# vivek-tiwari-vt/2048-Using-Reinforcement-Learning

Hardware: AMD Instinct MI355X
Metric: board-steps/sec (batched env.step) (higher is better)
Workload: dtype u8 (packed log2 tiles; f64 reward arithmetic, f32 reward out)

## Files before the change

2048-using-reinforcement-learning_amd/csrc/g2048_board.h:

```cpp
#pragma once
#include <stdint.h>

#if defined(__HIPCC__)
#include <hip/hip_runtime.h>
#define G2048_HD __device__ __forceinline__
#define G2048_PERM(s0, s1, sel) __builtin_amdgcn_perm((s0), (s1), (sel))
#define G2048_UDOT4(a, b, c) __builtin_amdgcn_udot4((a), (b), (c), false)
#else
#define G2048_HD inline
#if !defined(G2048_PERM) || !defined(G2048_UDOT4)
#error "host builds of g2048_board.h (test harness only) must define G2048_PERM and G2048_UDOT4"
#endif
#endif

namespace g2048 {

struct Board { uint32_t w[4]; };

constexpr uint32_t B80 = 0x80808080u;
constexpr uint32_t B7F = 0x7f7f7f7fu;

enum : uint32_t { DOM_STEP = 1, DOM_RESET = 2, DOM_BEAM = 3, DOM_SYNTH_BOARD = 4, DOM_SYNTH_ACTION = 5, DOM_EPISODE = 6, DOM_POLICY = 7,
                  DOM_SIMULATE = 8, DOM_MINIBATCH = 9, DOM_REPLAY = 10 };

// ... 199 lines not shown
        uint32_t g;
        const Board d = move_agent(b, 3u, g, false);
        m = (m & 7u) | (same(d, b) ? 0u : 8u);
    }
    return m;
}

G2048_HD bool game_over(const Board &b) { return valid_mask_env(b) == 0u; }

G2048_HD uint32_t spawn_rowprefix(Board &b, uint32_t h, bool enable = true, uint32_t *zf_out = nullptr)
{
    const uint32_t ones = 0x01010101u;
    const uint32_t z0 = zflag(b.w[0]), z1 = zflag(b.w[1]), z2 = zflag(b.w[2]), z3 = zflag(b.w[3]);
    const uint32_t c0 = popc(z0), c1 = c0 + popc(z1), c2 = c1 + popc(z2), n = c2 + popc(z3);
    const uint32_t idx = ((h >> 16) * n) >> 16;
    const uint32_t row = (idx >= c0 ? 1u : 0u) + (idx >= c1 ? 1u : 0u) + (idx >= c2 ? 1u : 0u);
    const uint32_t z = row == 0 ? z0 : row == 1 ? z1 : row == 2 ? z2 : z3;
    const uint32_t k1 = idx + 1u - (row == 0 ? 0u : row == 1 ? c0 : row == 2 ? c1 : c2);
    const uint32_t hit = zflag(((z >> 7) * ones) ^ (enable ? k1 * ones : 0x7f7f7f7fu)) & z;
    const uint32_t add = hit >> (((h & 0xffffu) >= 58982u) ? 6 : 7);
    b.w[0] |= row == 0 ? add : 0u; b.w[1] |= row == 1 ? add : 0u;
    b.w[2] |= row == 2 ? add : 0u; b.w[3] |= row == 3 ? add : 0u;
    if (zf_out) {
        zf_out[0] = z0 ^ (row == 0 ? hit : 0u); zf_out[1] = z1 ^ (row == 1 ? hit : 0u);
        zf_out[2] = z2 ^ (row == 2 ? hit : 0u); zf_out[3] = z3 ^ (row == 3 ? hit : 0u);
    }
    return n;
}

G2048_HD uint32_t spawn_prefix(Board &b, uint32_t h, bool enable = true, uint32_t *zf_out = nullptr)
{
    const uint32_t ones = 0x01010101u;
    const uint32_t z0 = zflag(b.w[0]), z1 = zflag(b.w[1]), z2 = zflag(b.w[2]), z3 = zflag(b.w[3]);
    const uint32_t p0 = (z0 >> 7) * ones, p1 = (z1 >> 7) * ones, p2 = (z2 >> 7) * ones, p3 = (z3 >> 7) * ones;
    const uint32_t c0 = p0 >> 24, c1 = c0 + (p1 >> 24), c2 = c1 + (p2 >> 24), n = c2 + (p3 >> 24);
    const uint32_t idx = ((h >> 16) * n) >> 16;
    uint32_t t_on = (idx + 1u) * ones;
#if defined(__HIPCC__)
    asm volatile("" : "+v"(t_on));
#endif
    const uint32_t target = enable ? t_on : 0x7f7f7f7fu;
    const uint32_t h0 = zflag(p0 ^ target) & z0;
    const uint32_t h1 = zflag((p1 + c0 * ones) ^ target) & z1;
    const uint32_t h2 = zflag((p2 + c1 * ones) ^ target) & z2;
    const uint32_t h3 = zflag((p3 + c2 * ones) ^ target) & z3;
    const uint32_t sh = ((h & 0xffffu) >= 58982u) ? 6u : 7u;
    b.w[0] |= h0 >> sh; b.w[1] |= h1 >> sh; b.w[2] |= h2 >> sh; b.w[3] |= h3 >> sh;
    if (zf_out) { zf_out[0] = z0 ^ h0; zf_out[1] = z1 ^ h1; zf_out[2] = z2 ^ h2; zf_out[3] = z3 ^ h3; }
    return n;
}

G2048_HD Board fresh_board(uint32_t h0, uint32_t h1)
{
    const uint32_t cell0 = h0 >> 28;
    uint32_t cell1 = ((h1 >> 16) * 15u) >> 16;
    cell1 += cell1 >= cell0 ? 1u : 0u;
    const uint32_t code0 = (h0 & 0xffffu) >= 58982u ? 2u : 1u, code1 = (h1 & 0xffffu) >= 58982u ? 2u : 1u;
    const uint32_t t0 = code0 << (8u * (cell0 & 3u)), t1 = code1 << (8u * (cell1 & 3u));
    const uint32_t r0 = cell0 >> 2, r1 = cell1 >> 2;
    Board b;
#pragma unroll
    for (uint32_t r = 0; r < 4; ++r) b.w[r] = (r0 == r ? t0 : 0u) | (r1 == r ? t1 : 0u);
    return b;
}

G2048_HD uint32_t rng_draw(uint32_t k0, uint32_t k1, uint64_t id, uint32_t ctr)
{
    uint32_t h = (uint32_t)id ^ k0;
    h ^= h >> 16; h *= 0x85EBCA6Bu; h ^= h >> 13; h *= 0xC2B2AE35u; h ^= h >> 16;
    h += k1 + (uint32_t)(id >> 32) * 0x9E3779B1u + ctr * 0x85EBCA77u;
    h ^= h >> 16; h *= 0x7FEB352Du; h ^= h >> 15; h *= 0x846CA68Bu; h ^= h >> 16;
    return h;
}

G2048_HD uint32_t rng_draw_lo(uint32_t k0, uint32_t k1h, uint32_t id_lo, uint32_t ctr)
{
    uint32_t h = id_lo ^ k0;
    h ^= h >> 16; h *= 0x85EBCA6Bu; h ^= h >> 13; h *= 0xC2B2AE35u; h ^= h >> 16;
// ... 67 lines not shown
    const uint32_t v01 = geflag(cur.w[1], cur.w[0]) & n0 & n1;
    const uint32_t v12 = geflag(cur.w[2], cur.w[1]) & n1 & n2;
    const uint32_t v23 = geflag(cur.w[3], cur.w[2]) & n2 & n3;
    const uint32_t colcnt = (v01 >> 7) + (v12 >> 7) + (v23 >> 7);
#pragma unroll
    for (int i = 0; i < 4; ++i) {
        const uint32_t x = cur.w[i], n = i == 0 ? n0 : i == 1 ? n1 : i == 2 ? n2 : n3;
        const uint32_t h = geflag(x >> 8, x) & n & (n >> 8);
        const uint32_t c = popc(h) + ((colcnt >> (8 * i)) & 0xffu);
        r += (double)c * 0.1;
    }
    return r;
}

G2048_HD double reward_env(const Board &cur, const TileStats &st, uint32_t gain, bool valid,
                           uint32_t empty_before, uint32_t empty_after)
{
    return reward_env_from((double)gain / 4.0, cur, st, valid, empty_before, empty_after);
}

struct TenthByProduct {
    static constexpr uint32_t kColShift = 7u;
    G2048_HD double operator()(uint32_t rows, uint32_t cols) const { return (double)(rows + cols) * 0.1; }
    G2048_HD double crowded(double r, uint32_t empty_after) const { return empty_after <= 2u ? r - 2.0 : r; }
};

#define G2048_TENTHS 8
#define G2048_TENTHS_INIT { 0.0 * 0.1, 1.0 * 0.1, 2.0 * 0.1, 3.0 * 0.1, 4.0 * 0.1, 5.0 * 0.1, 6.0 * 0.1, 7.0 * 0.1 }
#define G2048_CROWDED 17
#define G2048_CROWDED_INIT { -2.0, -2.0, -2.0, 0.0, 0.0, 0.0, 0.0, 0.0, 0.0, 0.0, 0.0, 0.0, 0.0, 0.0, 0.0, 0.0, 0.0 }

template <class TENTH = TenthByProduct>
G2048_HD double reward_env_folded(const Board &cur, const TileStats &st, uint32_t gain, bool valid,
                                  uint32_t empty_before, uint32_t empty_after, TENTH tenth = TENTH())
{
    const int32_t q = (int32_t)gain - (valid ? 0 : 8) + 2 * ((int32_t)empty_after - (int32_t)empty_before);
    double r = (double)q * 0.25;
    r += div_small_ints((double)st.edge, (double)st.total) * 1.0;
    r = tenth.crowded(r, empty_after);
    const uint32_t n0 = nzflag(cur.w[0]), n1 = nzflag(cur.w[1]), n2 = nzflag(cur.w[2]), n3 = nzflag(cur.w[3]);
    const uint32_t v01 = geflag(cur.w[1], cur.w[0]) & n0 & n1;
    const uint32_t v12 = geflag(cur.w[2], cur.w[1]) & n1 & n2;
    const uint32_t v23 = geflag(cur.w[3], cur.w[2]) & n2 & n3;
    const uint32_t colcnt = (v01 >> TENTH::kColShift) + (v12 >> TENTH::kColShift) + (v23 >> TENTH::kColShift);
#pragma unroll
    for (int i = 0; i < 4; ++i) {
        const uint32_t x = cur.w[i], n = i == 0 ? n0 : i == 1 ? n1 : i == 2 ? n2 : n3;
        const uint32_t h = geflag(x >> 8, x) & n & (n >> 8);
        r += tenth(popc(h), (colcnt >> (8 * i)) & 0xffu);
    }
    return r;
}

G2048_HD uint32_t pair_count(const Board &b);
G2048_HD bool game_over_counted(const Board &b, uint32_t n_empty)
{
#if defined(__HIPCC__)
    const bool full = n_empty == 0u;
    uint32_t pairs = 1u;
    if (__builtin_amdgcn_ballot_w64(full) != 0ull) pairs = pair_count(b);
    return n_empty == 16u || (full && pairs == 0u);
#else
    if (n_empty == 16u) return true;
    if (n_empty != 0u) return false;
    return pair_count(b) == 0u;
#endif
}

struct StepOut { Board board; uint32_t gain; double reward; uint32_t flags; };

template <class MOVE, class TENTH = TenthByProduct>
G2048_HD StepOut step_board_with(const Board &prev, MOVE move, uint32_t h, TENTH tenth = TENTH())
{
    StepOut o;
    uint32_t merges;
    Board cur = move(prev, o.gain, merges);
    const bool valid = !same(cur, prev);
    uint32_t empty_mid;
    uint32_t zf[4];
    empty_mid = spawn_prefix(cur, h, valid, zf);
    const uint32_t empty_before = empty_mid - merges;
    const uint32_t empty_after = empty_mid - (valid ? 1u : 0u);
    const TileStats st = tile_stats_z(cur, empty_after, zf[0], zf[1], zf[2], zf[3]);
    o.reward = reward_env_folded(cur, st, o.gain, valid, empty_before, empty_after, tenth);
    const bool done = game_over_counted(cur, empty_after);
    const uint32_t maxcode = 31u - (uint32_t)__builtin_clz(st.orbits | 1u);
    o.flags = (done ? 1u : 0u) | (valid ? 2u : 0u) | (maxcode << 3);
    o.board = cur;
    return o;
}

G2048_HD StepOut step_board(const Board &prev, uint32_t action, uint32_t h)
{
    return step_board_with(prev, [action](const Board &b, uint32_t &g, uint32_t &m) { return move_env(b, action, g, m); }, h);
}

template <class TENTH = TenthByProduct>
G2048_HD StepOut step_board_sel_noop(const Board &prev, const DirSel &sel, bool noop, uint32_t h, TENTH tenth = TENTH())
{
    return step_board_with(prev, [&sel, noop](const Board &b, uint32_t &g, uint32_t &m) {
        const Board r = move_env_sel(b, sel, g, m);
        g = noop ? 0u : g; m = noop ? 0u : m;
        return Board{{noop ? b.w[0] : r.w[0], noop ? b.w[1] : r.w[1], noop ? b.w[2] : r.w[2], noop ? b.w[3] : r.w[3]}};
    }, h, tenth);
}

template <class TENTH = TenthByProduct>
G2048_HD StepOut step_board_sel(const Board &prev, const DirSel &sel, uint32_t h, TENTH tenth = TENTH())
{
    return step_board_with(prev, [&sel](const Board &b, uint32_t &g, uint32_t &m) { return move_env_sel(b, sel, g, m); }, h, tenth);
}

G2048_HD uint32_t sample_action(float p0, float p1, float p2, float p3, uint32_t mask4, uint32_t h, float &prob)
{
    const uint32_t m = (mask4 & 15u) ? (mask4 & 15u) : 15u;
    const float w0 = (m & 1u) ? p0 + 1e-10f : 0.0f, w1 = (m & 2u) ? p1 + 1e-10f : 0.0f;
    const float w2 = (m & 4u) ? p2 + 1e-10f : 0.0f, w3 = (m & 8u) ? p3 + 1e-10f : 0.0f;
// ... 275 lines not shown
```

2048-using-reinforcement-learning_amd/csrc/g2048_kernels.hip:

```cpp
#include <hip/hip_runtime.h>
#include <hip/hip_fp16.h>
#include <stddef.h>

#include "../../include/g2048.h"
#include "../../include/g2048_testing.h"
#include "g2048_board.h"
#include "g2048_host.h"
#include "g2048_instrument.h"
#include "g2048_rng.h"

using namespace g2048;

namespace {

enum { KB_STEP = 0, KB_EPISODE = 2, KB_BEAM = 4, KB_POLICY = 6, KB_INDEX = 8 };

constexpr int kBlock = 256;
constexpr int kStepBoardsPerLane = 1;

__device__ const uint32_t kDirTable[G2048_DIR_TABLE_WORDS] = G2048_DIR_TABLE_INIT;

#include "g2048_step_table.h"

__device__ __forceinline__ void dir_table_to_lds(uint4 *s_dir)
{
    const uint32_t l = threadIdx.x & (G2048_DIR_TABLE_WORDS - 1u);
    reinterpret_cast<uint32_t *>(s_dir)[l] = kDirTable[l];
}

__device__ __forceinline__ DirSel dir_sel(const uint4 *s_dir, uint32_t action)
{
    const uint4 i = s_dir[2u * action], o = s_dir[2u * action + 1u];
    return DirSel{i.x, i.y, i.z, i.w, o.x, o.y, o.z, o.w};
}

__device__ __forceinline__ Board load_board(const uint4 *p, size_t i)
{
    const uint4 v = p[i];
    return Board{{v.x, v.y, v.z, v.w}};
}

__device__ __forceinline__ void store_board(uint4 *p, size_t i, const Board &b)
// ... 484 lines not shown

__global__ void keys_advance_kernel(uint32_t *keyblock, unsigned long long *counter, uint64_t seed)
{
    const uint64_t idx = *counter;
    const Keys s = rng_keys(seed, DOM_STEP, idx), e = rng_keys(seed, DOM_EPISODE, idx);
    const Keys b = rng_keys(seed, DOM_BEAM, idx), p = rng_keys(seed, DOM_POLICY, idx);
    keyblock[KB_STEP] = s.k0; keyblock[KB_STEP + 1] = s.k1; keyblock[KB_EPISODE] = e.k0; keyblock[KB_EPISODE + 1] = e.k1;
    keyblock[KB_BEAM] = b.k0; keyblock[KB_BEAM + 1] = b.k1; keyblock[KB_POLICY] = p.k0; keyblock[KB_POLICY + 1] = p.k1;
    keyblock[KB_INDEX] = (uint32_t)idx; keyblock[KB_INDEX + 1] = (uint32_t)(idx >> 32);
    *counter = idx + 1ull;
}

__global__ void selftest_kernel(uint32_t *result, uint32_t a, uint32_t b, double x, double y, double z)
{
    uint32_t bad = 0;
    if (perm(a, b, 0x07040300u) != (((a >> 24) << 24) | ((a & 0xffu) << 16) | ((b >> 24) << 8) | (b & 0xffu))) bad |= 1u;
    if (perm(a, b, 0x0c0c0c05u) != ((a >> 8) & 0xffu)) bad |= 2u;
    if (dot4(a, b, 7u) != 7u + (a & 0xffu) * (b & 0xffu) + ((a >> 8) & 0xffu) * ((b >> 8) & 0xffu) +
                              ((a >> 16) & 0xffu) * ((b >> 16) & 0xffu) + (a >> 24) * (b >> 24)) bad |= 4u;
    if (x * y + z != 0.0) bad |= 8u;
    const Board c = {{0x03020100u, 0x07060504u, 0x0b0a0908u, 0x0f0e0d0cu}};
    const Board t = transpose(c);
    if (t.w[0] != 0x0c080400u || t.w[1] != 0x0d090501u || t.w[2] != 0x0e0a0602u || t.w[3] != 0x0f0b0703u) bad |= 16u;
    const Board r = rot180(c);
    if (r.w[0] != 0x0c0d0e0fu || r.w[3] != 0x00010203u) bad |= 32u;
    *result = bad;
}

struct StepBound {
    const uint4 *in; const uint8_t *actions; uint4 *out; uint32_t *score; void *reward; uint8_t *flags;
    size_t n; uint32_t id_lo, id_hi_term;
};

struct StepCall { uint64_t magic; StepBound b; uint64_t seed; uint32_t opts, per_lane, grid, reserved; };
static_assert(sizeof(StepCall) <= G2048_STEP_CALL_BYTES, "the caller's block holds a StepCall");
constexpr uint64_t kStepCallMagic = 0x6b63617038343032ull;

constexpr uint32_t kStepOpts = G2048_STEP_REWARD_F64 | G2048_STEP_AUTO_RESET | G2048_STEP_RANDOM_ACTIONS | G2048_STEP_NOOP_ACTIONS |
                               (3u << G2048_STEP_TUNE_SHIFT);

int step_check(const char *what, const void *boards_in, const uint8_t *actions, const void *boards_out, const uint32_t *score_inout,
               const void *reward_out, const uint8_t *flags_out, uint32_t opts)
{
    const bool random_actions = (opts & G2048_STEP_RANDOM_ACTIONS) != 0u;
    if (!boards_in || (!actions && !random_actions) || !boards_out || !score_inout || !reward_out || !flags_out)
        return fail(G2048_ERR_ARG, "%s: null pointer", what);
    if (!aligned(boards_in, 16) || !aligned(boards_out, 16)) return fail(G2048_ERR_ARG, "%s: board arrays must be 16-byte aligned", what);
    if (!aligned(score_inout, 4) || !aligned(reward_out, (opts & G2048_STEP_REWARD_F64) ? 8 : 4))
        return fail(G2048_ERR_ARG, "%s: score/reward arrays misaligned", what);
    if (opts & ~kStepOpts) return fail(G2048_ERR_ARG, "%s: unknown opts 0x%x", what, opts);
    if (((opts >> G2048_STEP_TUNE_SHIFT) & 3u) == 3u)
        return fail(G2048_ERR_ARG, "%s: tune 3 (four boards per lane) was removed: measured slower at every size", what);
    return G2048_OK;
}

int step_boards_per_lane(uint32_t opts, size_t n)
{
    const unsigned tune = (opts >> G2048_STEP_TUNE_SHIFT) & 3u;
    return tune == 1 ? 1 : tune == 2 ? 2 : (n >= ((size_t)1 << 22) ? 2 : kStepBoardsPerLane);
}

template <class Kernel>
void launch_step(Kernel kernel, unsigned grid, hipStream_t s, const StepBound &b, const uint32_t *keyblock, const Keys &k, const Keys &e,
                 uint32_t a0 = 0, uint32_t a1 = 0)
{
    hipLaunchKernelGGL(kernel, dim3(grid), dim3(kBlock), 0, s, b.n, keyblock, b.in, b.actions, b.score, b.id_lo, b.id_hi_term, k.k0, k.k1, b.out,
                       b.reward, b.flags, e.k0, e.k1, a0, a1);
}

void launch_plain_step(bool f64, bool ar, int per_lane, unsigned grid, hipStream_t s, const StepBound &b, const uint32_t *keyblock,
                       const Keys &k, const Keys &e);

}

extern "C" {

const char *g2048_last_error(void) { return g_err; }
int g2048_abi_version(void) { return G2048_ABI_VERSION; }
unsigned g2048_build_flags(void) { return kInstrument; }

int g2048_device_count(void)
{
    int n = 0;
    if (hipGetDeviceCount(&n) != hipSuccess) { (void)hipGetLastError(); return 0; }
    return n;
}

static int step_impl(const void *boards_in, const uint8_t *actions, void *boards_out, uint32_t *score_inout,
                     void *reward_out, uint8_t *flags_out, uint64_t seed, uint64_t step_index,
                     uint64_t board_id_base, size_t n, uint32_t opts, void *stream, const uint32_t *keyblock)
{
    if (n == 0) return G2048_OK;
    const bool random_actions = (opts & G2048_STEP_RANDOM_ACTIONS) != 0u;
    if (const int rc = step_check("g2048_step", boards_in, actions, boards_out, score_inout, reward_out, flags_out, opts)) return rc;
    {
        const uint64_t to_wrap = 0x100000000ull - (board_id_base & 0xffffffffull);
        if ((uint64_t)n > to_wrap) {
            const size_t n1 = (size_t)to_wrap, rb = (opts & G2048_STEP_REWARD_F64) ? 8u : 4u;
            const int rc = step_impl(boards_in, actions, boards_out, score_inout, reward_out, flags_out, seed, step_index, board_id_base, n1,
                                     opts, stream, keyblock);
            if (rc != G2048_OK) return rc;
            return step_impl(static_cast<const char *>(boards_in) + 16u * n1, actions ? actions + n1 : nullptr,
                             static_cast<char *>(boards_out) + 16u * n1, score_inout + n1, static_cast<char *>(reward_out) + rb * n1,
                             flags_out + n1, seed, step_index, board_id_base + n1, n - n1, opts, stream, keyblock);
// ... 1 lines not shown
    }
    if (random_actions && keyblock) return fail(G2048_ERR_ARG, "g2048_step_dyn: RANDOM_ACTIONS needs the scalar form");
    const Keys k = rng_keys(seed, DOM_STEP, step_index), e = rng_keys(seed, DOM_EPISODE, step_index);
    hipStream_t s = static_cast<hipStream_t>(stream);
    const StepBound b = {static_cast<const uint4 *>(boards_in), actions, static_cast<uint4 *>(boards_out), score_inout, reward_out, flags_out,
                         n, (uint32_t)board_id_base, rng_hi_term(board_id_base)};
    const bool f64 = opts & G2048_STEP_REWARD_F64, ar = opts & G2048_STEP_AUTO_RESET;
    const int per_lane = step_boards_per_lane(opts, n);
    if (opts & G2048_STEP_NOOP_ACTIONS) {
        if (random_actions) return fail(G2048_ERR_ARG, "g2048_step: NOOP_ACTIONS needs explicit actions");
        with_bools(f64, ar, [&](auto F, auto A) {
            launch_step(step_kernel<decltype(F)::value, decltype(A)::value, 1, kBlock, false, true>, blocks_for(n, kBlock), s, b, keyblock, k, e);
        });
    } else if (random_actions) {
        const Keys ak = rng_keys(seed, DOM_SYNTH_ACTION, step_index);
        with_bools(f64, ar, [&](auto F, auto A) {
            launch_step(step_kernel<decltype(F)::value, decltype(A)::value, 1, kBlock, true>, blocks_for(n, kBlock), s, b, keyblock, k, e, ak.k0, ak.k1);
        });
    } else {
        launch_plain_step(f64, ar, per_lane, blocks_for(n, (size_t)kBlock * per_lane), s, b, keyblock, k, e);
    }
    return check_launch("g2048_step");
}

namespace {
void launch_plain_step(bool f64, bool ar, int per_lane, unsigned grid, hipStream_t s, const StepBound &b, const uint32_t *keyblock,
                       const Keys &k, const Keys &e)
{
    with_bools(f64, ar, [&](auto F, auto A) {
        if (per_lane == 1) launch_step(step_kernel<decltype(F)::value, decltype(A)::value, 1, kBlock>, grid, s, b, keyblock, k, e);
        else launch_step(step_kernel<decltype(F)::value, decltype(A)::value, 2, kBlock>, grid, s, b, keyblock, k, e);
    });
}
}

int g2048_step(const void *boards_in, const uint8_t *actions, void *boards_out, uint32_t *score_inout,
               void *reward_out, uint8_t *flags_out, uint64_t seed, uint64_t step_index,
               uint64_t board_id_base, size_t n, uint32_t opts, void *stream)
{
    return step_impl(boards_in, actions, boards_out, score_inout, reward_out, flags_out, seed, step_index, board_id_base, n,
                     opts, stream, nullptr);
}

int g2048_step_pack(const void *boards_in, const uint8_t *actions, void *boards_out, uint32_t *score_inout, void *reward_out,
                    uint8_t *flags_out, uint64_t seed, uint64_t board_id_base, size_t n, uint32_t opts, void *call_out)
{
    if (!call_out || !aligned(call_out, 8)) return fail(G2048_ERR_ARG, "g2048_step_pack: call_out must be an 8-byte aligned block of G2048_STEP_CALL_BYTES");
    static_cast<StepCall *>(call_out)->magic = 0;
    if (const int rc = step_check("g2048_step_pack", boards_in, actions, boards_out, score_inout, reward_out, flags_out, opts)) return rc;
    if (opts & (G2048_STEP_RANDOM_ACTIONS | G2048_STEP_NOOP_ACTIONS))
        return fail(G2048_ERR_ARG, "g2048_step_pack: RANDOM_ACTIONS and NOOP_ACTIONS go through g2048_step");
    if ((uint64_t)n > 0x100000000ull - (board_id_base & 0xffffffffull))
        return fail(G2048_ERR_ARG, "g2048_step_pack: the board ids cross a multiple of 2^32 (two launches): use g2048_step");
    const int per_lane = step_boards_per_lane(opts, n);
    StepCall c = {};
    c.b = StepBound{static_cast<const uint4 *>(boards_in), actions, static_cast<uint4 *>(boards_out), score_inout, reward_out, flags_out,
                    n, (uint32_t)board_id_base, rng_hi_term(board_id_base)};
    c.seed = seed; c.opts = opts; c.per_lane = (uint32_t)per_lane; c.grid = blocks_for(n, (size_t)kBlock * per_lane);
    c.magic = kStepCallMagic;
    *static_cast<StepCall *>(call_out) = c;
    return G2048_OK;
}

int g2048_step_packed(const void *call, uint64_t step_index, void *stream)
{
    const StepCall *c = static_cast<const StepCall *>(call);
    if (!c || !aligned(c, 8) || c->magic != kStepCallMagic) return fail(G2048_ERR_ARG, "g2048_step_packed: not a block g2048_step_pack filled");
    if (c->b.n == 0) return G2048_OK;
    launch_plain_step(c->opts & G2048_STEP_REWARD_F64, c->opts & G2048_STEP_AUTO_RESET, (int)c->per_lane, c->grid, static_cast<hipStream_t>(stream),
                      c->b, nullptr, rng_keys(c->seed, DOM_STEP, step_index), rng_keys(c->seed, DOM_EPISODE, step_index));
    return check_launch("g2048_step_packed");
}

int g2048_step_dyn(const void *boards_in, const uint8_t *actions, void *boards_out, uint32_t *score_inout,
                   void *reward_out, uint8_t *flags_out, const uint32_t *keyblock, uint64_t board_id_base, size_t n,
                   uint32_t opts, void *stream)
{
    if (!keyblock) return fail(G2048_ERR_ARG, "g2048_step_dyn: null key block");
    return step_impl(boards_in, actions, boards_out, score_inout, reward_out, flags_out, 0, 0, board_id_base, n, opts, stream,
                     keyblock);
}

int g2048_step_many(const void *boards_in, const uint8_t *actions_stream_or_null, void *boards_out, uint32_t *score_inout,
                    void *reward_stream_out_or_null, uint8_t *flags_stream_out_or_null, uint8_t *flags_last_out,
                    uint32_t *episodes_out_or_null, uint64_t seed, uint64_t step_index0, uint32_t steps,
                    uint64_t board_id_base, size_t n, uint32_t opts, void *stream)
{
    if (n == 0) return G2048_OK;
    if (!boards_in || !boards_out || !score_inout || !flags_last_out) return fail(G2048_ERR_ARG, "g2048_step_many: null pointer");
    if (!aligned(boards_in, 16) || !aligned(boards_out, 16)) return fail(G2048_ERR_ARG, "g2048_step_many: board arrays must be 16-byte aligned");
    const bool f64 = (opts & G2048_STEP_REWARD_F64) != 0u, ar = (opts & G2048_STEP_AUTO_RESET) != 0u;
    const bool random_actions = (opts & G2048_STEP_RANDOM_ACTIONS) != 0u;
    if (!aligned(score_inout, 4) || !aligned(episodes_out_or_null, 4) || !aligned(reward_stream_out_or_null, f64 ? 8 : 4))
        return fail(G2048_ERR_ARG, "g2048_step_many: score / reward / episode arrays misaligned");
    if (!random_actions && !actions_stream_or_null)
        return fail(G2048_ERR_ARG, "g2048_step_many: no policy: pass an actions stream or set G2048_STEP_RANDOM_ACTIONS");
    if (opts & ~(G2048_STEP_REWARD_F64 | G2048_STEP_AUTO_RESET | G2048_STEP_RANDOM_ACTIONS)) return fail(G2048_ERR_ARG, "g2048_step_many: unknown opts 0x%x", opts);
    if (steps == 0) return fail(G2048_ERR_ARG, "g2048_step_many: steps must be at least 1");
    hipStream_t s = static_cast<hipStream_t>(stream);
    const auto launch = [&](auto kernel) {
        hipLaunchKernelGGL(kernel, dim3(blocks_for(n, kBlock)), dim3(kBlock), 0, s, static_cast<const uint4 *>(boards_in), actions_stream_or_null,
                           static_cast<uint4 *>(boards_out), score_inout, reward_stream_out_or_null, flags_stream_out_or_null, flags_last_out,
                           episodes_out_or_null, seed, step_index0, steps, board_id_base, n);
    };
// ... 281 lines not shown
```

2048-using-reinforcement-learning_amd/g2048/_build.py:

```python
import os
import shutil
import subprocess
import sys

CSRC = os.path.join(os.path.dirname(os.path.dirname(os.path.abspath(__file__))), "csrc")
INCLUDE = os.path.join(CSRC, "..", "..", "include")
LIBRARIES = {
    "": ("libg2048_hip.so", "G2048_LIB",
         ["g2048_kernels.hip", "g2048_beam.hip", "g2048_rollout.hip", "g2048_policy.hip", "g2048_tpolicy.hip", "g2048_qnet.hip",
          "g2048_qnet_batch.hip", "g2048_qnet_grad.hip", "g2048_qnet_step.hip", "g2048_per.hip", "g2048_ppo_grad.hip", "g2048_ppo_step.hip"],
         ["g2048.h", "g2048_testing.h"]),
    "TRAIN_": ("libg2048_train_hip.so", "G2048_TRAIN_LIB", ["g2048_qnet_train.hip"], ["g2048_train.h"]),
    "TLEARN_": ("libg2048_tlearn_hip.so", "G2048_TLEARN_LIB", ["g2048_tpolicy_grad.hip"], ["g2048_tlearn.h"]),
    "TSTEP_": ("libg2048_tstep_hip.so", "G2048_TSTEP_LIB", ["g2048_tpolicy_step.hip"], ["g2048_tstep.h"]),
    "TTRAIN_": ("libg2048_ttrain_hip.so", "G2048_TTRAIN_LIB", ["g2048_tpolicy_train.hip"], ["g2048_ttrain.h"]),
}
EXTENSIONS = {
    "COLLECT_": ("libg2048_collect_hip.so", "G2048_COLLECT_LIB", ["g2048_qnet_collect.hip"], ["g2048_collect.h"]),
}
PPO_EXTENSIONS = {
    "PPO_COLLECT_": ("libg2048_ppo_collect_hip.so", "G2048_PPO_COLLECT_LIB", ["g2048_ppo_collect.hip"], ["g2048_ppo_collect.h"]),
}
ROWS = {**LIBRARIES, **EXTENSIONS, **PPO_EXTENSIONS}
EXTRA_ROWS = {
    "TPOLICY_COLLECT_": ("libg2048_tpolicy_collect_hip.so", "G2048_TPOLICY_COLLECT_LIB", ["g2048_tpolicy_collect.hip"],
                         ["g2048_tpolicy_collect.h"]),
    "TBF16_": ("libg2048_tbf16_hip.so", "G2048_TBF16_LIB", ["g2048_tpolicy_bf16.hip"], ["g2048_tbf16.h"]),
    "SEARCH_": ("libg2048_search_hip.so", "G2048_SEARCH_LIB", ["g2048_expectimax.hip"], ["g2048_search.h"]),
}
ALL_ROWS = {**ROWS, **EXTRA_ROWS}
PUBLIC_HEADERS = [os.path.join(INCLUDE, h) for row in ALL_ROWS.values() for h in row[3]]
for _key, (_file, _env, _sources, _) in ALL_ROWS.items():
    globals()[_key + "LIB"] = os.environ.get(_env) or os.path.join(CSRC, _file)
    globals()[_key + "SOURCES"] = _sources
FLAGS = ["--offload-arch=gfx950", "-O3", "-std=c++17", "-fPIC", "-shared", "-ffp-contract=off", "-fvisibility=hidden",
         "-mllvm", "-amdgpu-kernarg-preload-count=16",
         "-Wl,--version-script=" + os.path.join(CSRC, "g2048_exports.map"), "-Wall", "-Wno-unused-function"]


def path_of(key):
    return globals()[key + "LIB"]


def _stale(lib):
    if not os.path.exists(lib):
        return True
    t = os.path.getmtime(lib)
    deps = [os.path.join(CSRC, f) for f in os.listdir(CSRC) if f.endswith((".hip", ".h", ".inc", ".hpp", ".map"))] + PUBLIC_HEADERS
    return any(os.path.exists(d) and os.path.getmtime(d) > t for d in deps)


def needs_build():
    return any(_stale(path_of(key)) for key in ALL_ROWS)


def build_one(key, lib=None, extra_flags=(), verbose=False):
    hipcc = shutil.which("hipcc") or "/opt/rocm/bin/hipcc"
    out = lib or path_of(key)
    srcs = [os.path.join(CSRC, f) for f in ALL_ROWS[key][2] if os.path.exists(os.path.join(CSRC, f))]
    cmd = [hipcc] + FLAGS + list(extra_flags) + ["-o", out] + srcs
    if verbose:
        print(" ".join(cmd))
    subprocess.check_call(cmd)
    return out


def build(force=False, verbose=False, lib=None, extra_flags=()):
    if lib is not None:
        return build_one("", lib, extra_flags, verbose)
    for key in ALL_ROWS:
        if force or _stale(path_of(key)):
            build_one(key, None, extra_flags, verbose)
    return path_of("")


if __name__ == "__main__":
    out, args = None, sys.argv[1:]
    key = next((k for k in ALL_ROWS if k and args[:1] == ["--" + k[:-1].lower().replace("_", "-")]), None)
    if key:
        args = args[1:]
    if args[:1] == ["-o"]:
        out, args = args[1], args[2:]
    if key:
        print(build_one(key, lib=out, extra_flags=args, verbose=True))
    else:
        print(build(force=True, verbose=True, lib=out, extra_flags=args))
```

2048-using-reinforcement-learning_amd/g2048/ops.py:

```python
import ctypes as C

import torch

from . import _lib as L


def _dev(t):
    return t.device


class KeyBlock:

    def __init__(self, seed, start=0, device="cuda"):
        self.seed = int(seed)
        self.device = torch.device(device)
        self.words = torch.zeros(L.KEYBLOCK_WORDS, dtype=torch.int32, device=self.device)
        self.counter = torch.full((1,), int(start), dtype=torch.int64, device=self.device)

    def advance(self):
        L.call(self.device, L.lib().g2048_keys_advance, self.words.data_ptr(), self.counter.data_ptr(), L.u64(self.seed),
               L.stream_ptr(self.device))
        return self


def _require_scores(scores):
    L.require_device_tensor(scores, torch.uint32 if scores.dtype == torch.uint32 else torch.int32, None, "scores")


def _output(t, n, dtype, tail, name, device):
    if t is None:
        return torch.empty((n,) + tuple(tail or ()), dtype=dtype, device=device)
    L.require_device_tensor(t, dtype, tail, name)
    if tail is not None and t.shape[0] != n:
        raise ValueError("g2048: %s must have n %s" % (name, "rows" if tail else "entries"))
    return t


# ... 74 lines not shown
            raise ValueError("g2048: random actions need the scalar (seed, step_index) form")
        actions = boards
    else:
        L.require_device_tensor(actions, torch.uint8, None, "actions")
    _require_scores(scores)
    if actions.shape[0] != n or scores.shape[0] != n:
        raise ValueError("g2048: actions/scores length must equal the number of boards")
    dev = _dev(boards)
    if out is None:
        out = torch.empty_like(boards)
    rdt = torch.float64 if reward_f64 else torch.float32
    if reward is None:
        reward = torch.empty(n, dtype=rdt, device=dev)
    if flags is None:
        flags = torch.empty(n, dtype=torch.uint8, device=dev)
    L.require_device_tensor(out, torch.uint8, (16,), "out")
    L.require_device_tensor(reward, rdt, None, "reward")
    L.require_device_tensor(flags, torch.uint8, None, "flags")
    opts = ((L.STEP_REWARD_F64 if reward_f64 else 0) | (L.STEP_AUTO_RESET if auto_reset else 0) |
            (L.STEP_RANDOM_ACTIONS if random_actions else 0) | (L.STEP_NOOP_ACTIONS if noop_actions else 0) | ((int(tune) & 3) << 8))
    act_ptr = None if random_actions else actions.data_ptr()
    if keyblock is not None:
        L.call(dev, L.lib().g2048_step_dyn, boards.data_ptr(), act_ptr, out.data_ptr(), scores.data_ptr(),
               reward.data_ptr(), flags.data_ptr(), keyblock.words.data_ptr(), L.u64(id_base), n, opts, L.stream_ptr(dev))
    else:
        L.call(dev, L.lib().g2048_step, boards.data_ptr(), act_ptr, out.data_ptr(), scores.data_ptr(),
               reward.data_ptr(), flags.data_ptr(), L.u64(seed), L.u64(step_index), L.u64(id_base), n, opts,
               L.stream_ptr(dev))
    return out, reward, flags


class PreparedStep:

    def __init__(self, boards, actions, scores, seed, id_base=0, *, out, reward, flags, auto_reset=False, tune=0):
        step(boards, actions, scores, seed, 0, id_base, out=out, reward=reward, flags=flags,
             reward_f64=reward.dtype == torch.float64, auto_reset=auto_reset, tune=tune)
        self._keep = (boards, actions, scores, out, reward, flags)
        self.device = boards.device
        opts = ((L.STEP_REWARD_F64 if reward.dtype == torch.float64 else 0) | (L.STEP_AUTO_RESET if auto_reset else 0) |
                ((int(tune) & 3) << 8))
        head = (boards.data_ptr(), actions.data_ptr(), out.data_ptr(), scores.data_ptr(), reward.data_ptr(), flags.data_ptr(),
                L.u64(seed))
        tail = (L.u64(id_base), boards.shape[0], opts)
        self._block = (L.C.c_uint64 * (L.STEP_CALL_BYTES // 8))()
        self._call = L.C.addressof(self._block)
        self.packed = L.lib().g2048_step_pack(*head, *tail, self._call) == L.OK
        if self.packed:
            self._fn = L.lib().g2048_step_packed
        else:
            self._fn, self._head, self._tail = L.lib().g2048_step, head, tail

    def __call__(self, step_index, stream_ptr=None):
        if stream_ptr is None:
            stream_ptr = torch.cuda.current_stream(self.device).cuda_stream
        if self.packed:
            rc = self._fn(self._call, int(step_index), stream_ptr)
        else:
            rc = self._fn(*self._head, int(step_index), *self._tail, stream_ptr)
        if rc != L.OK:
            L.check(rc)


class StepChains:

    ALIGN = 256

    def __init__(self, n, chains, device="cuda"):
        n, chains = int(n), int(chains)
        if chains < 1:
            raise ValueError("g2048: chains must be at least 1")
        self.device = torch.device(device)
        per = -(-max(n, 1) // chains)
        per = -(-per // self.ALIGN) * self.ALIGN
        self.bounds = [(lo, min(lo + per, n)) for lo in range(0, max(n, 1), per)]
        self._side = None
        self._events = None
        self._open_on = None
        self._held = []

    def __len__(self):
        return len(self.bounds)

    @property
# ... 1688 lines not shown
```

Baseline: 125.6 billion.

## Cut step launch overhead with native Python call object and module launch; trim spawn math

Adds a C-extension StepCall object so the prepared step skips ctypes argument marshalling, and launches the kernel through a cached hipFunction_t with a prebuilt kernarg image via hipModuleLaunchKernel. On the device side it folds the prefix-count offsets into the spawn multiplies, reuses the zero flags for the reward's nonzero masks, and replaces the full-board pair count in game-over detection with a cheaper any-pair test. The extra native extension adds build complexity, and the launch path now relies on the kernel parameter layout matching a hand-declared signature.

```diff
diff --git a/2048-using-reinforcement-learning_amd/csrc/g2048_board.h b/2048-using-reinforcement-learning_amd/csrc/g2048_board.h
--- a/2048-using-reinforcement-learning_amd/csrc/g2048_board.h
+++ b/2048-using-reinforcement-learning_amd/csrc/g2048_board.h
@@ -255,8 +255,10 @@
 {
     const uint32_t ones = 0x01010101u;
     const uint32_t z0 = zflag(b.w[0]), z1 = zflag(b.w[1]), z2 = zflag(b.w[2]), z3 = zflag(b.w[3]);
-    const uint32_t p0 = (z0 >> 7) * ones, p1 = (z1 >> 7) * ones, p2 = (z2 >> 7) * ones, p3 = (z3 >> 7) * ones;
-    const uint32_t c0 = p0 >> 24, c1 = c0 + (p1 >> 24), c2 = c1 + (p2 >> 24), n = c2 + (p3 >> 24);
+    const uint32_t p0 = (z0 >> 7) * ones, c0 = p0 >> 24;
+    const uint32_t p1 = ((z1 >> 7) + c0) * ones, c1 = p1 >> 24;
+    const uint32_t p2 = ((z2 >> 7) + c1) * ones, c2 = p2 >> 24;
+    const uint32_t p3 = ((z3 >> 7) + c2) * ones, n = p3 >> 24;
     const uint32_t idx = ((h >> 16) * n) >> 16;
     uint32_t t_on = (idx + 1u) * ones;
 #if defined(__HIPCC__)
@@ -264,9 +266,9 @@
 #endif
     const uint32_t target = enable ? t_on : 0x7f7f7f7fu;
     const uint32_t h0 = zflag(p0 ^ target) & z0;
-    const uint32_t h1 = zflag((p1 + c0 * ones) ^ target) & z1;
-    const uint32_t h2 = zflag((p2 + c1 * ones) ^ target) & z2;
-    const uint32_t h3 = zflag((p3 + c2 * ones) ^ target) & z3;
+    const uint32_t h1 = zflag(p1 ^ target) & z1;
+    const uint32_t h2 = zflag(p2 ^ target) & z2;
+    const uint32_t h3 = zflag(p3 ^ target) & z3;
     const uint32_t sh = ((h & 0xffffu) >= 58982u) ? 6u : 7u;
     b.w[0] |= h0 >> sh; b.w[1] |= h1 >> sh; b.w[2] |= h2 >> sh; b.w[3] |= h3 >> sh;
     if (zf_out) { zf_out[0] = z0 ^ h0; zf_out[1] = z1 ^ h1; zf_out[2] = z2 ^ h2; zf_out[3] = z3 ^ h3; }
@@ -400,13 +402,14 @@
 
 template <class TENTH = TenthByProduct>
 G2048_HD double reward_env_folded(const Board &cur, const TileStats &st, uint32_t gain, bool valid,
-                                  uint32_t empty_before, uint32_t empty_after, TENTH tenth = TENTH())
+                                  uint32_t empty_before, uint32_t empty_after, TENTH tenth = TENTH(), const uint32_t *zf = nullptr)
 {
     const int32_t q = (int32_t)gain - (valid ? 0 : 8) + 2 * ((int32_t)empty_after - (int32_t)empty_before);
     double r = (double)q * 0.25;
     r += div_small_ints((double)st.edge, (double)st.total) * 1.0;
     r = tenth.crowded(r, empty_after);
-    const uint32_t n0 = nzflag(cur.w[0]), n1 = nzflag(cur.w[1]), n2 = nzflag(cur.w[2]), n3 = nzflag(cur.w[3]);
+    const uint32_t n0 = zf ? zf[0] ^ B80 : nzflag(cur.w[0]), n1 = zf ? zf[1] ^ B80 : nzflag(cur.w[1]);
+    const uint32_t n2 = zf ? zf[2] ^ B80 : nzflag(cur.w[2]), n3 = zf ? zf[3] ^ B80 : nzflag(cur.w[3]);
     const uint32_t v01 = geflag(cur.w[1], cur.w[0]) & n0 & n1;
     const uint32_t v12 = geflag(cur.w[2], cur.w[1]) & n1 & n2;
     const uint32_t v23 = geflag(cur.w[3], cur.w[2]) & n2 & n3;
@@ -421,17 +424,28 @@
 }
 
 G2048_HD uint32_t pair_count(const Board &b);
+G2048_HD uint32_t any_pair_full(const Board &b)
+{
+    uint32_t w = 0u;
+#pragma unroll
+    for (int r = 0; r < 4; ++r) {
+        if (r < 3) w |= ~((b.w[r] ^ b.w[r + 1]) + B7F);
+        w |= ~((b.w[r] ^ (b.w[r] >> 8)) + B7F);
+    }
+    return w & B80;
+}
+
 G2048_HD bool game_over_counted(const Board &b, uint32_t n_empty)
 {
 #if defined(__HIPCC__)
     const bool full = n_empty == 0u;
     uint32_t pairs = 1u;
-    if (__builtin_amdgcn_ballot_w64(full) != 0ull) pairs = pair_count(b);
+    if (__builtin_amdgcn_ballot_w64(full) != 0ull) pairs = any_pair_full(b);
     return n_empty == 16u || (full && pairs == 0u);
 #else
     if (n_empty == 16u) return true;
     if (n_empty != 0u) return false;
-    return pair_count(b) == 0u;
+    return any_pair_full(b) == 0u;
 #endif
 }
 
@@ -450,7 +464,7 @@
     const uint32_t empty_before = empty_mid - merges;
     const uint32_t empty_after = empty_mid - (valid ? 1u : 0u);
     const TileStats st = tile_stats_z(cur, empty_after, zf[0], zf[1], zf[2], zf[3]);
-    o.reward = reward_env_folded(cur, st, o.gain, valid, empty_before, empty_after, tenth);
+    o.reward = reward_env_folded(cur, st, o.gain, valid, empty_before, empty_after, tenth, zf);
     const bool done = game_over_counted(cur, empty_after);
     const uint32_t maxcode = 31u - (uint32_t)__builtin_clz(st.orbits | 1u);
     o.flags = (done ? 1u : 0u) | (valid ? 2u : 0u) | (maxcode << 3);
diff --git a/2048-using-reinforcement-learning_amd/csrc/g2048_kernels.hip b/2048-using-reinforcement-learning_amd/csrc/g2048_kernels.hip
--- a/2048-using-reinforcement-learning_amd/csrc/g2048_kernels.hip
+++ b/2048-using-reinforcement-learning_amd/csrc/g2048_kernels.hip
@@ -1,6 +1,8 @@
 #include <hip/hip_runtime.h>
 #include <hip/hip_fp16.h>
 #include <stddef.h>
+
+#include <atomic>
 
 #include "../../include/g2048.h"
 #include "../../include/g2048_testing.h"
@@ -8,6 +10,7 @@
 #include "g2048_host.h"
 #include "g2048_instrument.h"
 #include "g2048_rng.h"
+#include "g2048_step_call.h"
 
 using namespace g2048;
 
@@ -558,10 +561,6 @@
     size_t n; uint32_t id_lo, id_hi_term;
 };
 
-struct StepCall { uint64_t magic; StepBound b; uint64_t seed; uint32_t opts, per_lane, grid, reserved; };
-static_assert(sizeof(StepCall) <= G2048_STEP_CALL_BYTES, "the caller's block holds a StepCall");
-constexpr uint64_t kStepCallMagic = 0x6b63617038343032ull;
-
 constexpr uint32_t kStepOpts = G2048_STEP_REWARD_F64 | G2048_STEP_AUTO_RESET | G2048_STEP_RANDOM_ACTIONS | G2048_STEP_NOOP_ACTIONS |
                                (3u << G2048_STEP_TUNE_SHIFT);
 
@@ -596,6 +595,18 @@
 
 void launch_plain_step(bool f64, bool ar, int per_lane, unsigned grid, hipStream_t s, const StepBound &b, const uint32_t *keyblock,
                        const Keys &k, const Keys &e);
+hipFunction_t plain_step_function(bool f64, bool ar, int per_lane);
+
+constexpr int kStepFnDevices = 64;
+std::atomic<hipFunction_t> g_step_fn[kStepFnDevices][8];
+
+template <class Kernel>
+hipFunction_t step_function_of(Kernel kernel)
+{
+    static_assert(same_parameters(Kernel{}, static_cast<StepKernelFn *>(nullptr)), "g2048_step_call.h lays out step_kernel's own parameter list");
+    hipFunction_t f = nullptr;
+    return hipGetFuncBySymbol(&f, reinterpret_cast<const void *>(kernel)) == hipSuccess ? f : nullptr;
+}
 
 }
 
@@ -663,6 +674,22 @@
         else launch_step(step_kernel<decltype(F)::value, decltype(A)::value, 2, kBlock>, grid, s, b, keyblock, k, e);
     });
 }
+
+hipFunction_t plain_step_function(bool f64, bool ar, int per_lane)
+{
+    int dev = 0;
+    if (hipGetDevice(&dev) != hipSuccess) return nullptr;
+    const bool cached = dev >= 0 && dev < kStepFnDevices;
+    const int slot = (f64 ? 1 : 0) | (ar ? 2 : 0) | (per_lane == 1 ? 0 : 4);
+    hipFunction_t f = cached ? g_step_fn[dev][slot].load(std::memory_order_acquire) : nullptr;
+    if (f) return f;
+    f = with_bools(f64, ar, [&](auto F, auto A) {
+        return per_lane == 1 ? step_function_of(step_kernel<decltype(F)::value, decltype(A)::value, 1, kBlock>)
+                             : step_function_of(step_kernel<decltype(F)::value, decltype(A)::value, 2, kBlock>);
+    });
+    if (f && cached) g_step_fn[dev][slot].store(f, std::memory_order_release);
+    return f;
+}
 }
 
 int g2048_step(const void *boards_in, const uint8_t *actions, void *boards_out, uint32_t *score_inout,
@@ -685,8 +712,8 @@
         return fail(G2048_ERR_ARG, "g2048_step_pack: the board ids cross a multiple of 2^32 (two launches): use g2048_step");
     const int per_lane = step_boards_per_lane(opts, n);
     StepCall c = {};
-    c.b = StepBound{static_cast<const uint4 *>(boards_in), actions, static_cast<uint4 *>(boards_out), score_inout, reward_out, flags_out,
-                    n, (uint32_t)board_id_base, rng_hi_term(board_id_base)};
+    kStepArgs.fill(c.image, n, nullptr, static_cast<const uint4 *>(boards_in), actions, score_inout, (uint32_t)board_id_base,
+                   rng_hi_term(board_id_base), 0u, 0u, static_cast<uint4 *>(boards_out), reward_out, flags_out, 0u, 0u, 0u, 0u);
     c.seed = seed; c.opts = opts; c.per_lane = (uint32_t)per_lane; c.grid = blocks_for(n, (size_t)kBlock * per_lane);
     c.magic = kStepCallMagic;
     *static_cast<StepCall *>(call_out) = c;
@@ -697,10 +724,15 @@
 {
     const StepCall *c = static_cast<const StepCall *>(call);
     if (!c || !aligned(c, 8) || c->magic != kStepCallMagic) return fail(G2048_ERR_ARG, "g2048_step_packed: not a block g2048_step_pack filled");
-    if (c->b.n == 0) return G2048_OK;
-    launch_plain_step(c->opts & G2048_STEP_REWARD_F64, c->opts & G2048_STEP_AUTO_RESET, (int)c->per_lane, c->grid, static_cast<hipStream_t>(stream),
-                      c->b, nullptr, rng_keys(c->seed, DOM_STEP, step_index), rng_keys(c->seed, DOM_EPISODE, step_index));
-    return check_launch("g2048_step_packed");
+    if (c->grid == 0) return G2048_OK;
+    const hipFunction_t f = plain_step_function(c->opts & G2048_STEP_REWARD_F64, c->opts & G2048_STEP_AUTO_RESET, (int)c->per_lane);
+    if (!f) return fail(G2048_ERR_HIP, "g2048_step_packed: no module function for the step kernel: %s", hipGetErrorString(hipGetLastError()));
+    alignas(8) unsigned char image[kStepImageBytes];
+    step_call_image(*c, step_index, image);
+    size_t bytes = kStepImageBytes;
+    void *config[] = {HIP_LAUNCH_PARAM_BUFFER_POINTER, image, HIP_LAUNCH_PARAM_BUFFER_SIZE, &bytes, HIP_LAUNCH_PARAM_END};
+    return check_hip(hipModuleLaunchKernel(f, c->grid, 1, 1, kBlock, 1, 1, 0, static_cast<hipStream_t>(stream), nullptr, config),
+                     "g2048_step_packed");
 }
 
 int g2048_step_dyn(const void *boards_in, const uint8_t *actions, void *boards_out, uint32_t *score_inout,
diff --git a/2048-using-reinforcement-learning_amd/csrc/g2048_step_call.h b/2048-using-reinforcement-learning_amd/csrc/g2048_step_call.h
--- /dev/null
+++ b/2048-using-reinforcement-learning_amd/csrc/g2048_step_call.h
@@ -0,0 +1,69 @@
+#pragma once
+#include <hip/hip_runtime.h>
+#include <stddef.h>
+#include <stdint.h>
+#include <string.h>
+
+#include <type_traits>
+
+#include "../../include/g2048.h"
+#include "g2048_board.h"
+#include "g2048_rng.h"
+
+namespace g2048 {
+
+using StepKernelFn = void(size_t n, const uint32_t *keyblock, const uint4 *boards_in, const uint8_t *actions, uint32_t *score,
+                          uint32_t id_lo_base, uint32_t id_hi_term, uint32_t k0, uint32_t k1, uint4 *boards_out, void *reward_out,
+                          uint8_t *flags_out, uint32_t e0, uint32_t e1, uint32_t a0, uint32_t a1);
+enum StepArg { SA_N, SA_KEYBLOCK, SA_IN, SA_ACTIONS, SA_SCORE, SA_ID_LO, SA_ID_HI_TERM, SA_K0, SA_K1, SA_OUT, SA_REWARD, SA_FLAGS,
+               SA_E0, SA_E1, SA_A0, SA_A1, SA_COUNT };
+
+template <class F> struct KernargLayout;
+template <class... A>
+struct KernargLayout<void(A...)> {
+    static constexpr size_t kCount = sizeof...(A);
+    size_t offset[kCount], size[kCount], bytes;
+    constexpr KernargLayout() : offset{}, size{}, bytes(0)
+    {
+        const size_t sz[] = {sizeof(A)...}, al[] = {alignof(A)...};
+        size_t at = 0;
+        for (size_t i = 0; i < kCount; ++i) {
+            at = (at + al[i] - 1) / al[i] * al[i];
+            offset[i] = at; size[i] = sz[i];
+            at += sz[i];
+        }
+        bytes = at;
+    }
+    void fill(unsigned char *image, A... value) const
+    {
+        size_t i = 0;
+        ((memcpy(image + offset[i], &value, sizeof value), ++i), ...);
+    }
+};
+
+template <class... A>
+constexpr bool same_parameters(void (*)(A...), StepKernelFn *) { return std::is_same_v<void(A...), StepKernelFn>; }
+
+constexpr KernargLayout<StepKernelFn> kStepArgs{};
+static_assert(KernargLayout<StepKernelFn>::kCount == SA_COUNT, "StepArg names every parameter");
+constexpr size_t kStepImageBytes = 96;
+static_assert(kStepArgs.bytes == kStepImageBytes, "the image is the explicit argument segment");
+
+struct StepCall {
+    uint64_t magic;
+    alignas(8) unsigned char image[kStepImageBytes];
+    uint64_t seed;
+    uint32_t opts, per_lane, grid, reserved;
+};
+static_assert(sizeof(StepCall) == G2048_STEP_CALL_BYTES, "the caller's block holds a StepCall");
+constexpr uint64_t kStepCallMagic = 0x6b63617038343032ull;
+
+inline void step_call_image(const StepCall &c, uint64_t step_index, unsigned char *image)
+{
+    memcpy(image, c.image, kStepImageBytes);
+    const Keys k = rng_keys(c.seed, DOM_STEP, step_index), e = rng_keys(c.seed, DOM_EPISODE, step_index);
+    memcpy(image + kStepArgs.offset[SA_K0], &k.k0, 4); memcpy(image + kStepArgs.offset[SA_K1], &k.k1, 4);
+    memcpy(image + kStepArgs.offset[SA_E0], &e.k0, 4); memcpy(image + kStepArgs.offset[SA_E1], &e.k1, 4);
+}
+
+}
diff --git a/2048-using-reinforcement-learning_amd/csrc/g2048_stepcall_py.cpp b/2048-using-reinforcement-learning_amd/csrc/g2048_stepcall_py.cpp
--- /dev/null
+++ b/2048-using-reinforcement-learning_amd/csrc/g2048_stepcall_py.cpp
@@ -0,0 +1,170 @@
+#define PY_SSIZE_T_CLEAN
+#include <Python.h>
+#include <stddef.h>
+#include <stdint.h>
+#include <structmember.h>
+
+#include "../../include/g2048.h"
+
+namespace {
+
+using PackFn = int (*)(const void *, const uint8_t *, void *, uint32_t *, void *, uint8_t *, uint64_t, uint64_t, size_t, uint32_t, void *);
+using PackedFn = int (*)(const void *, uint64_t, void *);
+
+struct StepCallObject {
+    PyObject_HEAD
+    vectorcallfunc vectorcall;
+    PackedFn packed;
+    PyObject *check, *current_stream, *keep, *device;
+    alignas(8) unsigned char block[G2048_STEP_CALL_BYTES];
+};
+
+bool as_u64(PyObject *o, uint64_t *out)
+{
+    const unsigned long long v = PyLong_AsUnsignedLongLongMask(o);
+    if (v == (unsigned long long)-1 && PyErr_Occurred()) return false;
+    *out = (uint64_t)v;
+    return true;
+}
+
+PyObject *stepcall_vectorcall(PyObject *self_, PyObject *const *args, size_t nargsf, PyObject *kwnames)
+{
+    StepCallObject *self = reinterpret_cast<StepCallObject *>(self_);
+    const Py_ssize_t nargs = PyVectorcall_NARGS(nargsf);
+    if ((kwnames && PyTuple_GET_SIZE(kwnames) != 0) || nargs < 1 || nargs > 2) {
+        PyErr_SetString(PyExc_TypeError, "StepCall(step_index, stream_ptr=None) takes one or two positional arguments");
+        return nullptr;
+    }
+    uint64_t step_index, stream;
+    if (!as_u64(args[0], &step_index)) return nullptr;
+    if (nargs == 2 && args[1] != Py_None) {
+        if (!as_u64(args[1], &stream)) return nullptr;
+    } else {
+        PyObject *s = PyObject_CallNoArgs(self->current_stream);
+        if (!s) return nullptr;
+        const bool good = as_u64(s, &stream);
+        Py_DECREF(s);
+        if (!good) return nullptr;
+    }
+    const int rc = self->packed(self->block, step_index, reinterpret_cast<void *>(static_cast<uintptr_t>(stream)));
+    if (rc != G2048_OK) {
+        PyObject *r = PyObject_CallFunction(self->check, "i", rc);
+        if (!r) return nullptr;
+        Py_DECREF(r);
+        PyErr_Format(PyExc_RuntimeError, "g2048: g2048_step_packed returned status %d", rc);
+        return nullptr;
+    }
+    Py_RETURN_NONE;
+}
+
+PyObject *stepcall_new(PyTypeObject *type, PyObject *args, PyObject *kwargs)
+{
+    static const char *names[] = {"pack", "packed", "args", "check", "current_stream", "keep", "device", nullptr};
+    unsigned long long pack_at = 0, packed_at = 0;
+    PyObject *call_args, *check, *current_stream, *keep, *device;
+    if (!PyArg_ParseTupleAndKeywords(args, kwargs, "KKO!OOOO:StepCall", const_cast<char **>(names), &pack_at, &packed_at, &PyTuple_Type,
+                                     &call_args, &check, &current_stream, &keep, &device))
+        return nullptr;
+    if (!pack_at || !packed_at || PyTuple_GET_SIZE(call_args) != 10 || !PyCallable_Check(check) || !PyCallable_Check(current_stream)) {
+        PyErr_SetString(PyExc_TypeError, "StepCall: two entry-point addresses, g2048_step_pack's ten leading arguments, two callables");
+        return nullptr;
+    }
+    uint64_t a[10];
+    for (int i = 0; i < 10; ++i) {
+        PyObject *o = PyTuple_GET_ITEM(call_args, i);
+        a[i] = 0;
+        if (o != Py_None && !as_u64(o, &a[i])) return nullptr;
+    }
+    StepCallObject *self = reinterpret_cast<StepCallObject *>(type->tp_alloc(type, 0));
+    if (!self) return nullptr;
+    self->vectorcall = stepcall_vectorcall;
+    self->packed = reinterpret_cast<PackedFn>(static_cast<uintptr_t>(packed_at));
+    const auto ptr = [&](int i) { return reinterpret_cast<void *>(static_cast<uintptr_t>(a[i])); };
+    const int rc = reinterpret_cast<PackFn>(static_cast<uintptr_t>(pack_at))(
+        ptr(0), static_cast<const uint8_t *>(ptr(1)), ptr(2), static_cast<uint32_t *>(ptr(3)), ptr(4), static_cast<uint8_t *>(ptr(5)), a[6], a[7],
+        static_cast<size_t>(a[8]), static_cast<uint32_t>(a[9]), self->block);
+    if (rc != G2048_OK) {
+        Py_DECREF(self);
+        PyErr_Format(PyExc_ValueError, "g2048_step_pack refused the call (status %d)", rc);
+        return nullptr;
+    }
+    Py_INCREF(check); self->check = check;
+    Py_INCREF(current_stream); self->current_stream = current_stream;
+    Py_INCREF(keep); self->keep = keep;
+    Py_INCREF(device); self->device = device;
+    return reinterpret_cast<PyObject *>(self);
+}
+
+int stepcall_traverse(PyObject *self_, visitproc visit, void *arg)
+{
+    StepCallObject *self = reinterpret_cast<StepCallObject *>(self_);
+    Py_VISIT(self->check); Py_VISIT(self->current_stream); Py_VISIT(self->keep); Py_VISIT(self->device);
+    return 0;
+}
+
+int stepcall_clear(PyObject *self_)
+{
+    StepCallObject *self = reinterpret_cast<StepCallObject *>(self_);
+    Py_CLEAR(self->check); Py_CLEAR(self->current_stream); Py_CLEAR(self->keep); Py_CLEAR(self->device);
+    return 0;
+}
+
+void stepcall_dealloc(PyObject *self_)
+{
+    PyObject_GC_UnTrack(self_);
+    stepcall_clear(self_);
+    Py_TYPE(self_)->tp_free(self_);
+}
+
+PyObject *stepcall_packed(PyObject *, void *) { Py_RETURN_TRUE; }
+
+PyObject *stepcall_block(PyObject *self_, void *)
+{
+    StepCallObject *self = reinterpret_cast<StepCallObject *>(self_);
+    return PyBytes_FromStringAndSize(reinterpret_cast<const char *>(self->block), sizeof self->block);
+}
+
+PyMemberDef stepcall_members[] = {
+    {"device", T_OBJECT_EX, offsetof(StepCallObject, device), READONLY, "the device of the tensors the call is bound to"},
+    {"_keep", T_OBJECT_EX, offsetof(StepCallObject, keep), READONLY, "the tensors the call is bound to, kept alive"},
+    {nullptr, 0, 0, 0, nullptr},
+};
+
+PyGetSetDef stepcall_getset[] = {
+    {"packed", stepcall_packed, nullptr, "True: the call goes through g2048_step_packed", nullptr},
+    {"block", stepcall_block, nullptr, "a copy of the G2048_STEP_CALL_BYTES block", nullptr},
+    {nullptr, nullptr, nullptr, nullptr, nullptr},
+};
+
+PyTypeObject StepCallType = {PyVarObject_HEAD_INIT(nullptr, 0)};
+
+PyModuleDef module_def = {PyModuleDef_HEAD_INIT, "_stepcall", "native prepared step call (g2048_step_pack / g2048_step_packed)", -1, nullptr};
+
+}
+
+PyMODINIT_FUNC PyInit__stepcall(void)
+{
+    StepCallType.tp_name = "g2048._stepcall.StepCall";
+    StepCallType.tp_basicsize = sizeof(StepCallObject);
+    StepCallType.tp_flags = Py_TPFLAGS_DEFAULT | Py_TPFLAGS_HAVE_GC | Py_TPFLAGS_HAVE_VECTORCALL;
+    StepCallType.tp_vectorcall_offset = offsetof(StepCallObject, vectorcall);
+    StepCallType.tp_call = PyVectorcall_Call;
+    StepCallType.tp_new = stepcall_new;
+    StepCallType.tp_dealloc = stepcall_dealloc;
+    StepCallType.tp_traverse = stepcall_traverse;
+    StepCallType.tp_clear = stepcall_clear;
+    StepCallType.tp_members = stepcall_members;
+    StepCallType.tp_getset = stepcall_getset;
+    StepCallType.tp_doc = "g2048_step with everything but the step index and the stream bound once; call(step_index, stream_ptr=None)";
+    if (PyType_Ready(&StepCallType) < 0) return nullptr;
+    PyObject *m = PyModule_Create(&module_def);
+    if (!m) return nullptr;
+    Py_INCREF(&StepCallType);
+    if (PyModule_AddObject(m, "StepCall", reinterpret_cast<PyObject *>(&StepCallType)) < 0 ||
+        PyModule_AddIntConstant(m, "STEP_CALL_BYTES", G2048_STEP_CALL_BYTES) < 0) {
+        Py_DECREF(&StepCallType);
+        Py_DECREF(m);
+        return nullptr;
+    }
+    return m;
+}
diff --git a/2048-using-reinforcement-learning_amd/g2048/_build.py b/2048-using-reinforcement-learning_amd/g2048/_build.py
--- a/2048-using-reinforcement-learning_amd/g2048/_build.py
+++ b/2048-using-reinforcement-learning_amd/g2048/_build.py
@@ -2,6 +2,7 @@
 import shutil
 import subprocess
 import sys
+import sysconfig
 
 CSRC = os.path.join(os.path.dirname(os.path.dirname(os.path.abspath(__file__))), "csrc")
 INCLUDE = os.path.join(CSRC, "..", "..", "include")
@@ -38,6 +39,11 @@
          "-Wl,--version-script=" + os.path.join(CSRC, "g2048_exports.map"), "-Wall", "-Wno-unused-function"]
 
 
+STEPCALL_EXT = os.path.join(os.path.dirname(os.path.abspath(__file__)), "_stepcall.so")
+STEPCALL_SOURCE = os.path.join(CSRC, "g2048_stepcall_py.cpp")
+STEPCALL_FLAGS = ["-x", "c++", "-O2", "-std=c++17", "-fPIC", "-shared", "-fvisibility=hidden", "-Wall"]
+
+
 def path_of(key):
     return globals()[key + "LIB"]
 
@@ -50,8 +56,24 @@
     return any(os.path.exists(d) and os.path.getmtime(d) > t for d in deps)
 
 
+def _stepcall_stale():
+    if not os.path.exists(STEPCALL_EXT):
+        return True
+    t = os.path.getmtime(STEPCALL_EXT)
+    return any(os.path.getmtime(d) > t for d in (STEPCALL_SOURCE, os.path.join(INCLUDE, "g2048.h")))
+
+
 def needs_build():
-    return any(_stale(path_of(key)) for key in ALL_ROWS)
+    return any(_stale(path_of(key)) for key in ALL_ROWS) or _stepcall_stale()
+
+
+def build_stepcall(verbose=False):
+    hipcc = shutil.which("hipcc") or "/opt/rocm/bin/hipcc"
+    cmd = [hipcc] + STEPCALL_FLAGS + ["-I" + sysconfig.get_paths()["include"], "-o", STEPCALL_EXT, STEPCALL_SOURCE]
+    if verbose:
+        print(" ".join(cmd))
+    subprocess.check_call(cmd)
+    return STEPCALL_EXT
 
 
 def build_one(key, lib=None, extra_flags=(), verbose=False):
@@ -71,6 +93,8 @@
     for key in ALL_ROWS:
         if force or _stale(path_of(key)):
             build_one(key, None, extra_flags, verbose)
+    if force or _stepcall_stale():
+        build_stepcall(verbose)
     return path_of("")
 
 
diff --git a/2048-using-reinforcement-learning_amd/g2048/ops.py b/2048-using-reinforcement-learning_amd/g2048/ops.py
--- a/2048-using-reinforcement-learning_amd/g2048/ops.py
+++ b/2048-using-reinforcement-learning_amd/g2048/ops.py
@@ -3,6 +3,11 @@
 import torch
 
 from . import _lib as L
+
+try:
+    from . import _stepcall
+except ImportError:
+    _stepcall = None
 
 
 def _dev(t):
@@ -143,23 +148,33 @@
 
 class PreparedStep:
 
-    def __init__(self, boards, actions, scores, seed, id_base=0, *, out, reward, flags, auto_reset=False, tune=0):
+    def __new__(cls, boards, actions, scores, seed, id_base=0, *, out, reward, flags, auto_reset=False, tune=0):
         step(boards, actions, scores, seed, 0, id_base, out=out, reward=reward, flags=flags,
              reward_f64=reward.dtype == torch.float64, auto_reset=auto_reset, tune=tune)
-        self._keep = (boards, actions, scores, out, reward, flags)
-        self.device = boards.device
+        keep = (boards, actions, scores, out, reward, flags)
+        device = boards.device
         opts = ((L.STEP_REWARD_F64 if reward.dtype == torch.float64 else 0) | (L.STEP_AUTO_RESET if auto_reset else 0) |
                 ((int(tune) & 3) << 8))
         head = (boards.data_ptr(), actions.data_ptr(), out.data_ptr(), scores.data_ptr(), reward.data_ptr(), flags.data_ptr(),
                 L.u64(seed))
         tail = (L.u64(id_base), boards.shape[0], opts)
+        lib = L.lib()
+        if _stepcall is not None:
+            try:
+                return _stepcall.StepCall(L.C.cast(lib.g2048_step_pack, L.C.c_void_p).value, L.C.cast(lib.g2048_step_packed, L.C.c_void_p).value,
+                                          head + tail, L.check, lambda: torch.cuda.current_stream(device).cuda_stream, keep, device)
+            except ValueError:
+                pass
+        self = super().__new__(cls)
+        self._keep, self.device = keep, device
         self._block = (L.C.c_uint64 * (L.STEP_CALL_BYTES // 8))()
         self._call = L.C.addressof(self._block)
-        self.packed = L.lib().g2048_step_pack(*head, *tail, self._call) == L.OK
+        self.packed = lib.g2048_step_pack(*head, *tail, self._call) == L.OK
         if self.packed:
-            self._fn = L.lib().g2048_step_packed
+            self._fn = lib.g2048_step_packed
         else:
-            self._fn, self._head, self._tail = L.lib().g2048_step, head, tail
+            self._fn, self._head, self._tail = lib.g2048_step, head, tail
+        return self
 
     def __call__(self, step_index, stream_ptr=None):
         if stream_ptr is None:
```

Measured after the change: 131.8 billion (median of 6 runs). +4.9%, better.
